# supranational/sppark

Hardware: AMD Instinct MI355X
Metric: MSM points/sec (BLS12-381 G1, 2^26 points) (higher is better)
Workload: dtype u32

## Files before the change

### sppark_amd/csrc/ec/xyzzx_dev.hpp

```cpp
#pragma once
#include "../ff/montx_dev.hpp"
#include "xyzz_dev.hpp"

namespace sppark_amd {

template<class FP> struct field_is_internal { static constexpr bool value = false; };
template<class P, int LB> struct field_is_internal<montx_dev<P, LB>> { static constexpr bool value = true; };
template<class FP> struct field_is_montx { static constexpr bool value = false; };
template<class P, int LB> struct field_is_montx<montx_dev<P, LB>> { static constexpr bool value = true; };

template<class P, int LB> struct affine_loader<montx_dev<P, LB>> {
    typedef montx_dev<P, LB> F;
    static constexpr unsigned RAW = 2 * F::NL * 4;
    static constexpr unsigned STRIDE = RAW <= 64 ? 64 : RAW <= 128 ? 128 : ((RAW + 15) / 16) * 16;
    template<bool FLAGGED>
    SPPARK_DEVFN static affine_dev<F> load(const unsigned char* base, size_t idx, unsigned)
    {
        const uint4* q = reinterpret_cast<const uint4*>(base + idx * (size_t)STRIDE);
        u32 w[(RAW + 15) / 16 * 4];
        #pragma unroll
        for (unsigned i = 0; i < (RAW + 15) / 16; i++) { uint4 v = q[i]; w[4*i] = v.x; w[4*i+1] = v.y; w[4*i+2] = v.z; w[4*i+3] = v.w; }
        affine_dev<F> a;
        a.X = F::from_wire(w); a.Y = F::from_wire(w + F::NL);
        a.inf = (a.X.l[F::NL - 1] >> 31) != 0;
        a.X.l[F::NL - 1] &= 0x7fffffffu;
        return a;
    }
    template<bool FLAGGED>
    SPPARK_DEVFN static void convert(unsigned char* dst, const unsigned char* src, size_t idx, unsigned stride)
    {
        typedef mont_dev<P> S;
        u32 wx[S::N], wy[S::N];
        bool inf;
        if (!FLAGGED && (S::N % 2) == 0 && (stride & 15) == 0 && ((size_t)src & 15) == 0) {
            const uint4* q = reinterpret_cast<const uint4*>(src + idx * (size_t)stride);
            u32 w[2 * S::N];
            #pragma unroll
            for (int i = 0; i < S::N / 2; i++) { uint4 v = q[i]; w[4*i] = v.x; w[4*i+1] = v.y; w[4*i+2] = v.z; w[4*i+3] = v.w; }
            u32 any = 0;
            #pragma unroll
            for (int i = 0; i < S::N; i++) { wx[i] = w[i]; wy[i] = w[S::N + i]; any |= w[i] | w[S::N + i]; }
            inf = any == 0;
        } else {
            affine_dev<S> p = affine_loader<S>::template load<FLAGGED>(src, idx, stride);
            p.X.to_wire(wx); p.Y.to_wire(wy);
            inf = p.inf;
        }
        F x = F::from_std(wx), y = F::from_std(wy);
        u32 w[STRIDE / 4] = {};
        x.to_wire(w); y.to_wire(w + F::NL);
        if (inf) w[F::NL - 1] |= 0x80000000u;
        uint4* q = reinterpret_cast<uint4*>(dst + idx * (size_t)STRIDE);
        #pragma unroll
        for (unsigned i = 0; i < STRIDE / 16; i++) q[i] = make_uint4(w[4*i], w[4*i+1], w[4*i+2], w[4*i+3]);
    }
};

template<class P, int LB> struct xyzz_dev<montx_dev<P, LB>> {
    typedef montx_dev<P, LB> F;
    F X, Y, ZZZ, ZZ;
    static constexpr bool TIGHT = F::TIGHT;
    static constexpr int BX = TIGHT ? 1 : 6;
    static constexpr int BX2 = TIGHT ? 1 : 4;
    SPPARK_DEVFN static F keep_x(const F& x3) { if constexpr (TIGHT) return x3.norm(); else return x3; }
    SPPARK_DEVFN static F minus_y(const F& y) { if constexpr (TIGHT) return F::template neg<4, 2>(y); else return F::template neg<6, 4>(y); }

    SPPARK_DEVFN bool is_inf() const { return ZZ.limbs_all_zero(); }
    SPPARK_DEVFN void set_inf() { X = F::zero(); Y = F::zero(); ZZZ = F::zero(); ZZ = F::zero(); }

    SPPARK_DEVFN void set(const affine_dev<F>& p, bool negate)
    {
        if (p.inf) { set_inf(); return; }
        X = p.X; Y = negate ? F::template neg<3>(p.Y) : p.Y;
        ZZZ = F::one(); ZZ = F::one();
    }

    SPPARK_DEVFN void madd(const affine_dev<F>& p, bool negate)
    {
        if (p.inf) return;
        if (is_inf()) { set(p, negate); return; }

        F U2, S2;
        F::template mul2<true, true>(U2, S2, p.X, ZZ, p.Y, ZZZ);
        if (negate) S2 = F::template neg<3>(S2);
        F Pd = F::template sub<11, BX>(U2, X).norm();
        F Rd;
        if constexpr (TIGHT) Rd = F::template sub<4, 2>(S2, Y).norm(); else Rd = F::template sub<6, 4>(S2, Y).norm();

        if (!Pd.template is_zero_mod<13>()) {
            F PP, RR, PPP, Q;
            F::sqr2(PP, RR, Pd, Rd);
            F::template mul2<true, false>(PPP, Q, Pd, PP, X, PP);
            F T   = PPP + Q + Q;
            F X3  = keep_x(F::template sub<8, 3>(RR, T));
            F D   = F::template sub<11, BX>(Q, X3);
            F nY  = minus_y(Y);
            Y   = F::mul_add(D, Rd, nY, PPP);
            F::template mul2<true, true>(ZZ, ZZZ, ZZ, PP, ZZZ, PPP);
            X = X3;
        } else if (Rd.template is_zero_mod<9>()) {
            F y2 = negate ? F::template neg<3>(p.Y).norm() : p.Y;
            dbl_affine(p.X, y2);
        } else {
            set_inf();
        }
    }

    SPPARK_DEVFN void add(const xyzz_dev& q)
    {
        if (q.is_inf()) return;
        if (is_inf()) { *this = q; return; }

        F U1 = X * q.ZZ;
        F S1 = Y * q.ZZZ;
        F U2 = q.X * ZZ;
        F S2 = q.Y * ZZZ;
        F Pd = F::template sub<3>(U2, U1).norm();
        F Rd = F::template sub<3>(S2, S1).norm();

        if (!Pd.template is_zero_mod<5>()) {
            F PP  = Pd.sqr();
            F PPP = Pd * PP;
            F Q   = U1 * PP;
            F T   = PPP + Q + Q;
            F X3  = keep_x(F::template sub<8, 3>(Rd.sqr(), T));
            F D   = F::template sub<11, BX>(Q, X3);
            Y   = F::mul_add(D, Rd, F::template neg<3>(S1), PPP);
            ZZ  = (ZZ * PP) * q.ZZ;
            ZZZ = (ZZZ * PPP) * q.ZZZ;
            X = X3;
        } else if (Rd.template is_zero_mod<5>()) {
            xyzz_dev t = *this;
            dbl_outlined(t);
            *this = t;
        } else {
            set_inf();
        }
    }

    SPPARK_DEVFN void add_pairs(const xyzz_dev& q)
    {
        if (q.is_inf()) return;
        if (is_inf()) { *this = q; return; }
        F U1, S1, U2, S2;
        F::mul2(U1, S1, X, q.ZZ, Y, q.ZZZ);
        F::mul2(U2, S2, q.X, ZZ, q.Y, ZZZ);
        F Pd = F::template sub<3>(U2, U1).norm();
        F Rd = F::template sub<3>(S2, S1).norm();
        if (!Pd.template is_zero_mod<5>()) {
            F PP, RR, PPP, Q, t0, t1;
            F::sqr2(PP, RR, Pd, Rd);
            F::template mul2<true, true>(PPP, Q, Pd, PP, U1, PP);
            F T   = PPP + Q + Q;
            F X3  = keep_x(F::template sub<8, 3>(RR, T));
            F D   = F::template sub<11, BX>(Q, X3);
            Y   = F::mul_add(D, Rd, F::template neg<3>(S1), PPP);
            F::template mul2<true, true>(t0, t1, ZZ, PP, ZZZ, PPP);
            F::template mul2<true, true>(ZZ, ZZZ, t0, q.ZZ, t1, q.ZZZ);
            X = X3;
        } else if (Rd.template is_zero_mod<5>()) {
            xyzz_dev t = *this;
            dbl_outlined(t);
            *this = t;
        } else {
            set_inf();
        }
    }
    SPPARK_DEVFN void dbl_pairs()
    {
        if (is_inf()) return;
        F Yn = Y.norm(), Xn = X.norm();
        F U = (Yn + Yn).norm();
        F V, M, W, S, M3s;
        F::sqr2(V, M, U, Xn);
        F::template mul2<true, true>(W, S, U, V, Xn, V);
        F M3 = (M + M + M).norm();
        M3s = M3.sqr();
        F X3 = keep_x(F::template sub<5, 2>(M3s, S + S));
        F D  = F::template sub<8, BX2>(S, X3);
        Y = F::mul_add(D, M3, F::template neg<3>(W), Yn);
        F::template mul2<true, true>(ZZ, ZZZ, ZZ, V, ZZZ, W);
        X = X3;
    }

#if defined(SPPARK_HOST_EMULATION)
    static void dbl_outlined(xyzz_dev& t) { t.dbl(); }
#else
    __device__ __noinline__ static void dbl_outlined(xyzz_dev& t) { t.dbl(); }
#endif

    SPPARK_DEVFN void dbl()
    {
        if (is_inf()) return;
        F Yn = Y.norm(), Xn = X.norm();
        F U = (Yn + Yn).norm();
        F V = U.sqr();
        F W = U * V;
        F S = Xn * V;
        F M = Xn.sqr();
        F M3 = (M + M + M).norm();
        F X3 = keep_x(F::template sub<5, 2>(M3.sqr(), S + S));
        F D  = F::template sub<8, BX2>(S, X3);
        Y = F::mul_add(D, M3, F::template neg<3>(W), Yn);
        ZZ = ZZ * V; ZZZ = ZZZ * W;
        X = X3;
    }

    typedef xyzz_mem<F::N> mem_t;

    SPPARK_DEVFN void store(mem_t* dst) const
    {
        constexpr int N = F::N;
        u32 s[4 * N];
        X.to_wire(s); Y.to_wire(s + N); ZZZ.to_wire(s + 2 * N); ZZ.to_wire(s + 3 * N);
        uint4* d = reinterpret_cast<uint4*>(dst);
        #pragma unroll
        for (int i = 0; i < N; i++) d[i] = make_uint4(s[4*i], s[4*i+1], s[4*i+2], s[4*i+3]);
    }
    SPPARK_DEVFN static xyzz_dev load(const mem_t* src)
    {
        constexpr int N = F::N;
        u32 d[4 * N];
        const uint4* q = reinterpret_cast<const uint4*>(src);
        #pragma unroll
        for (int i = 0; i < N; i++) { uint4 w = q[i]; d[4*i] = w.x; d[4*i+1] = w.y; d[4*i+2] = w.z; d[4*i+3] = w.w; }
        xyzz_dev r;
        r.X = F::from_wire(d); r.Y = F::from_wire(d + N); r.ZZZ = F::from_wire(d + 2 * N); r.ZZ = F::from_wire(d + 3 * N);
        return r;
    }

    SPPARK_DEVFN void store_std(xyzz_mem<P::N>* dst) const
    {
        constexpr int N = P::N;
        u32 s[4 * N];
        if (is_inf()) { for (int i = 0; i < 4 * N; i++) s[i] = 0; }
        else { X.to_std(s); Y.to_std(s + N); ZZZ.to_std(s + 2 * N); ZZ.to_std(s + 3 * N); }
        uint4* d = reinterpret_cast<uint4*>(dst);
        #pragma unroll
        for (int i = 0; i < N; i++) d[i] = make_uint4(s[4*i], s[4*i+1], s[4*i+2], s[4*i+3]);
    }

private:
    SPPARK_DEVFN void dbl_affine(const F& x, const F& y)
    {
        F U = (y + y).norm();
        F V = U.sqr();
        F W = U * V;
        F S = x * V;
        F M = x.sqr();
        F M3 = (M + M + M).norm();
        F X3 = keep_x(F::template sub<5, 2>(M3.sqr(), S + S));
        F D  = F::template sub<8, BX2>(S, X3);
        Y = F::mul_add(D, M3, F::template neg<3>(W), y);
        X = X3; ZZ = V; ZZZ = W;
    }
};

}
```

### sppark_amd/csrc/msm/msm_kernels.hpp

```cpp
#pragma once
#include "../ec/xyzz_dev.hpp"
#include "../ec/xyzzx_dev.hpp"

namespace sppark_amd {

static constexpr u32 KEY_NONE = 0xffffffffu;


__host__ __device__ inline unsigned window_len(unsigned w, unsigned nwins, unsigned nbits)
{   return nbits / nwins + (w < nbits % nwins ? 1u : 0u);   }

template<class LimbFn>
SPPARK_DEVFN void recode_digits(u32* digits, size_t n, size_t i, LimbFn limb, bool flip,
                                unsigned nwins, unsigned nbits, unsigned w_begin = 0, unsigned w_count = ~0u)
{
    u32 carry = 0;
    const unsigned w_end = w_count > nwins - w_begin ? nwins : w_begin + w_count;
    for (unsigned w = 0, bit = 0; w < w_end; w++) {
        const unsigned len = window_len(w, nwins, nbits);
        const u32 half = 1u << (len - 1), full = 1u << len, mask = full - 1;
        const unsigned li = bit >> 5, sh = bit & 31;
        bit += len;
        u64 two = limb(li) | ((u64)limb(li + 1) << 32);
        u32 d = ((u32)(two >> sh) & mask) + carry;
        bool minus = d > half;
        carry = minus;
        d = minus ? full - d : d;
        if (w >= w_begin) digits[(size_t)(w - w_begin) * n + i] = d ? (d | ((u32)(minus != flip) << 31)) : 0;
    }
}

template<class FR>
SPPARK_DEVFN FR load_scalar_abs(const u32* scalars, size_t i, int mont, bool& flip)
{
    constexpr int N = FR::N;
    FR s;
    const uint4* src = reinterpret_cast<const uint4*>(scalars + i * N);
    #pragma unroll
    for (int k = 0; k < N / 4; k++) {
        uint4 q = src[k];
        s.v[4*k] = q.x; s.v[4*k+1] = q.y; s.v[4*k+2] = q.z; s.v[4*k+3] = q.w;
    }
    if (mont) s = s.from();
    FR neg = FR::modulus_minus(s);
    u32 bw = 0;
    #pragma unroll
    for (int k = 0; k < N; k++) (void)__builtin_subc(neg.v[k], s.v[k], bw, &bw);
    flip = bw != 0;
    return FR::select(flip, neg, s);
}

template<class FR>
__global__ __launch_bounds__(256)
void k_breakdown(u32* __restrict__ digits, const u32* __restrict__ scalars,
                 unsigned n, unsigned nwins, unsigned nbits, int mont, unsigned w_begin, unsigned w_count)
{
    constexpr int N = FR::N;
    __shared__ u32 limbs[N + 2][256];
    const unsigned tid = threadIdx.x;
    for (unsigned i = blockIdx.x * 256 + tid; i < n; i += gridDim.x * 256) {
        bool flip;
        FR s = load_scalar_abs<FR>(scalars, i, mont, flip);
        #pragma unroll
        for (int k = 0; k < N; k++) limbs[k][tid] = s.v[k];
        limbs[N][tid] = 0; limbs[N + 1][tid] = 0;
        recode_digits(digits, n, i, [&](unsigned k) { return limbs[k][tid]; }, flip, nwins, nbits, w_begin, w_count);
    }
}

template<class FP, bool FLAGGED>
SPPARK_DEVFN void accumulate_chunk(xyzz_mem<FP::N>* buckets, u32* rec_key, xyzz_mem<FP::N>* rec_pt,
                                   const unsigned char* points, unsigned stride,
                                   const u32* sorted, const u32* off,
                                   unsigned n, unsigned NB, unsigned L, unsigned chunks_per_win,
                                   unsigned chunk, unsigned w_local, unsigned w_base = 0)
{
    if (chunk >= chunks_per_win) return;
    const unsigned w = w_base + w_local;
    const size_t rec0 = ((size_t)w * chunks_per_win + chunk) * 2;
    const u32* o = off + (size_t)w_local * (NB + 1);
    const unsigned total = o[NB];
    unsigned p = chunk * L;
    if (p >= total) { rec_key[rec0] = KEY_NONE; rec_key[rec0 + 1] = KEY_NONE; return; }
    const unsigned end = total < p + L ? total : p + L;

    unsigned lo = 0, hi = NB;
    while (hi - lo > 1) {
        unsigned mid = (lo + hi) >> 1;
        if (o[mid] <= p) lo = mid; else hi = mid;
    }
    unsigned b = lo, next = o[b + 1];

    const u32* src = sorted + (size_t)w_local * n;
    xyzz_dev<FP> acc;
    bool first_run = true;
    u32 slot0_key = KEY_NONE;

    u32 e = src[p];
    affine_dev<FP> pt = load_affine<FP, FLAGGED>(points, e & 0x7fffffffu, stride);
    acc.set(pt, e >> 31);
    constexpr bool PREFETCH = field_is_montx<FP>::value;
    u32 e_next = 0, e_next2 = 0;
    affine_dev<FP> pt_next = pt;
    if (PREFETCH && p + 1 < end) { e_next = src[p + 1]; pt_next = load_affine<FP, FLAGGED>(points, e_next & 0x7fffffffu, stride); }
    if (PREFETCH && p + 2 < end) e_next2 = src[p + 2];
    for (p++; p < end; p++) {
        if (PREFETCH) {
            e = e_next; pt = pt_next;
            if (p + 1 < end) { e_next = e_next2; pt_next = load_affine<FP, FLAGGED>(points, e_next & 0x7fffffffu, stride); }
            if (p + 2 < end) e_next2 = src[p + 2];
        } else {
            e = src[p];
            pt = load_affine<FP, FLAGGED>(points, e & 0x7fffffffu, stride);
        }
        if (p == next) {
            const u32 key = w * NB + b;
            if (first_run) { acc.store(&rec_pt[rec0]); slot0_key = key; first_run = false; }
            else           acc.store(&buckets[key]);
            do { b++; next = o[b + 1]; } while (p == next);
            acc.set(pt, e >> 31);
        } else {
            acc.madd(pt, e >> 31);
        }
    }
    const u32 key = w * NB + b;
    if (first_run) { acc.store(&rec_pt[rec0]); rec_key[rec0] = key; rec_key[rec0 + 1] = KEY_NONE; }
    else           { acc.store(&rec_pt[rec0 + 1]); rec_key[rec0] = slot0_key; rec_key[rec0 + 1] = key; }
}

#ifndef SPPARK_G2_TWO_WAVES_MAX_N
# define SPPARK_G2_TWO_WAVES_MAX_N 20
#endif
template<class FP, bool FLAGGED>
__global__ __launch_bounds__(256, (field_is_internal<FP>::value && FP::N <= 10) ? 3 : (field_is_internal<FP>::value && FP::N <= SPPARK_G2_TWO_WAVES_MAX_N) ? 2 : 1)
void k_accumulate(xyzz_mem<FP::N>* __restrict__ buckets,
                  u32* __restrict__ rec_key, xyzz_mem<FP::N>* __restrict__ rec_pt,
                  const unsigned char* __restrict__ points, unsigned stride,
                  const u32* __restrict__ sorted, const u32* __restrict__ off,
                  unsigned n, unsigned NB, unsigned L, unsigned chunks_per_win, unsigned w_base)
{
    accumulate_chunk<FP, FLAGGED>(buckets, rec_key, rec_pt, points, stride, sorted, off, n, NB, L,
                                  chunks_per_win, blockIdx.x * blockDim.x + threadIdx.x, blockIdx.y, w_base);
}

template<class FP, bool FLAGGED>
SPPARK_DEVFN void bitmap_accumulate_item(u32* rec_key, xyzz_mem<FP::N>* rec_pt,
                                         const unsigned char* points, unsigned stride, unsigned npoints,
                                         const u32* bitmap, const u32* refmap, unsigned span_words, size_t t)
{
    const size_t nwords = ((size_t)npoints + 31) / 32;
    const size_t w0 = t * span_words;
    if (w0 >= nwords) return;
    xyzz_dev<FP> acc; acc.set_inf();
    for (size_t w = w0; w < w0 + span_words && w < nwords; w++) {
        u32 bits = bitmap[w], refs = refmap ? refmap[w] : 0;
        bits ^= refs; refs &= bits;
        if (w == nwords - 1 && (npoints & 31)) bits &= (1u << (npoints & 31)) - 1;
        while (bits) {
            const unsigned k = __builtin_ctz(bits);
            bits &= bits - 1;
            affine_dev<FP> p = load_affine<FP, FLAGGED>(points, w * 32 + k, stride);
            acc.madd(p, (refs >> k) & 1);
        }
    }
    acc.store(&rec_pt[t]); rec_key[t] = 0;
}
template<class FP, bool FLAGGED>
__global__ __launch_bounds__(256)
void k_bitmap_accumulate(u32* __restrict__ rec_key, xyzz_mem<FP::N>* __restrict__ rec_pt,
                         const unsigned char* __restrict__ points, unsigned stride, unsigned npoints,
                         const u32* __restrict__ bitmap, const u32* __restrict__ refmap, unsigned span_words)
{
    bitmap_accumulate_item<FP, FLAGGED>(rec_key, rec_pt, points, stride, npoints, bitmap, refmap, span_words,
                                        (size_t)blockIdx.x * blockDim.x + threadIdx.x);
}

static constexpr unsigned JOIN_WALK = 8;
template<class FP> SPPARK_DEVFN void bucket_add(xyzz_dev<FP>& a, const xyzz_dev<FP>& b);
template<class FP> SPPARK_DEVFN void bucket_add_fast(xyzz_dev<FP>& a, const xyzz_dev<FP>& b);

template<class FP>
SPPARK_DEVFN void join_runs_item(xyzz_mem<FP::N>* buckets, u32* out_key, const u32* in_key,
                                 const xyzz_mem<FP::N>* in_pt, unsigned nrec, u32* any_long, size_t t)
{
    size_t job_h[2], job_e[2]; u32 job_k[2]; unsigned njobs = 0;
    for (unsigned s = 0; s < 2; s++) {
        if (t == 0 && s == 0) continue;
        const size_t q = 2 * t - 1 + s;
        if (q >= nrec) break;
        const u32 k = in_key[q];
        if (k == KEY_NONE) { out_key[q] = KEY_NONE; continue; }
        size_t h = q; bool is_long = false;
        for (size_t i = q, none = 0; i-- > 0;) {
            const u32 ki = in_key[i];
            if (ki == KEY_NONE) { if (++none == 2) break; continue; }
            none = 0;
            if (ki != k) break;
            h = i;
            if (q - h > JOIN_WALK) { is_long = true; break; }
        }
        size_t e = h;
        if (!is_long) {
            bool ended = false;
            size_t i = h + 1;
            for (unsigned none = 0; i < nrec && i <= h + JOIN_WALK; i++) {
                const u32 ki = in_key[i];
                if (ki == KEY_NONE) { if (++none == 2) { ended = true; break; } continue; }
                none = 0;
                if (ki != k) { ended = true; break; }
                e = i;
            }
            if (i >= nrec) ended = true;
            is_long = !ended;
        }
        if (is_long) { out_key[q] = k; *any_long = 1; continue; }
        out_key[q] = KEY_NONE;
        if (q == h) { job_h[njobs] = h; job_e[njobs] = e; job_k[njobs] = k; njobs++; }
    }
    for (unsigned j = 0; j < njobs; j++) {
        const size_t h = job_h[j], e = job_e[j]; const u32 k = job_k[j];
        xyzz_dev<FP> acc = xyzz_dev<FP>::load(&in_pt[h]);
        for (size_t i = h + 1; i <= e; i++)
            if (in_key[i] == k) bucket_add<FP>(acc, xyzz_dev<FP>::load(&in_pt[i]));
        acc.store(&buckets[k]);
    }
}

template<class FP>
SPPARK_DEVFN void reduce_runs_chunk(xyzz_mem<FP::N>* buckets, u32* out_key, xyzz_mem<FP::N>* out_pt,
                                    const u32* in_key, const xyzz_mem<FP::N>* in_pt,
                                    unsigned nrec, unsigned F, unsigned nthreads, int last, unsigned t)
{
    if (t >= nthreads) return;
    const unsigned lo = t * F, hi = nrec < lo + F ? nrec : lo + F;
    const size_t rec0 = (size_t)t * 2;

    xyzz_dev<FP> acc;
    u32 cur = KEY_NONE, slot0_key = KEY_NONE;
    bool first_run = true;

    for (unsigned r = lo; r < hi; r++) {
        const u32 k = in_key[r];
        if (k == KEY_NONE) continue;
        if (k == cur) {
            bucket_add_fast<FP>(acc, xyzz_dev<FP>::load(&in_pt[r]));
        } else {
            if (cur != KEY_NONE) {
                if (first_run && !last) { acc.store(&out_pt[rec0]); slot0_key = cur; }
                else                    acc.store(&buckets[cur]);
                first_run = false;
            }
            cur = k;
            acc = xyzz_dev<FP>::load(&in_pt[r]);
        }
    }
    if (last) {
        if (cur != KEY_NONE) acc.store(&buckets[cur]);
        return;
    }
    if (cur == KEY_NONE)      { out_key[rec0] = KEY_NONE; out_key[rec0 + 1] = KEY_NONE; }
    else if (first_run)       { acc.store(&out_pt[rec0]); out_key[rec0] = cur; out_key[rec0 + 1] = KEY_NONE; }
    else                      { acc.store(&out_pt[rec0 + 1]); out_key[rec0] = slot0_key; out_key[rec0 + 1] = cur; }
}

template<class FP>
__global__ __launch_bounds__(256)
void k_reduce_runs(xyzz_mem<FP::N>* __restrict__ buckets,
                   u32* __restrict__ out_key, xyzz_mem<FP::N>* __restrict__ out_pt,
                   const u32* __restrict__ in_key, const xyzz_mem<FP::N>* __restrict__ in_pt,
                   unsigned nrec, unsigned F, unsigned nthreads, int last, const u32* __restrict__ skip)
{
    if (skip != nullptr && *skip == 0) return;
    reduce_runs_chunk<FP>(buckets, out_key, out_pt, in_key, in_pt, nrec, F, nthreads, last,
                          blockIdx.x * blockDim.x + threadIdx.x);
}

static constexpr unsigned REDUCE_TAIL_NT = 256;
template<class FP>
__global__ __launch_bounds__(REDUCE_TAIL_NT)
void k_reduce_tail(xyzz_mem<FP::N>* __restrict__ buckets, u32* key0, xyzz_mem<FP::N>* pt0, u32* key1, xyzz_mem<FP::N>* pt1,
                   unsigned nrec, unsigned F, const u32* __restrict__ skip)
{
    if (skip != nullptr && *skip == 0) return;
    u32 *ik = key0, *ok = key1; xyzz_mem<FP::N> *ip = pt0, *op = pt1;
    for (;;) {
        const unsigned nthreads = (nrec + F - 1) / F;
        const int last = nthreads == 1;
        reduce_runs_chunk<FP>(buckets, ok, op, ik, ip, nrec, F, nthreads, last, threadIdx.x);
        if (last) break;
        __threadfence_block();
        __syncthreads();
        nrec = 2 * nthreads;
        u32* tk = ik; ik = ok; ok = tk;
        xyzz_mem<FP::N>* tp = ip; ip = op; op = tp;
    }
}

template<class FP>
__global__ __launch_bounds__(256, 2)
void k_join_runs(xyzz_mem<FP::N>* __restrict__ buckets, u32* __restrict__ out_key, const u32* __restrict__ in_key,
                 const xyzz_mem<FP::N>* __restrict__ in_pt, unsigned nrec, u32* __restrict__ any_long)
{
    join_runs_item<FP>(buckets, out_key, in_key, in_pt, nrec, any_long, (size_t)blockIdx.x * blockDim.x + threadIdx.x);
}

#if defined(SPPARK_HOST_EMULATION)
# define SPPARK_OUTLINED inline
#else
# define SPPARK_OUTLINED __device__ __noinline__
#endif
template<class FP> SPPARK_OUTLINED void xyzz_add_outlined(xyzz_dev<FP>& a, const xyzz_dev<FP>& b) { a.add(b); }
template<class FP> SPPARK_OUTLINED void xyzz_dbl_outlined(xyzz_dev<FP>& a) { a.dbl(); }
template<class FP> SPPARK_DEVFN void bucket_add(xyzz_dev<FP>& a, const xyzz_dev<FP>& b)
{   if constexpr (FP::N > 16) xyzz_add_outlined<FP>(a, b); else a.add(b);   }
template<class FP> SPPARK_DEVFN void bucket_dbl(xyzz_dev<FP>& a)
{   if constexpr (FP::N > 16) xyzz_dbl_outlined<FP>(a); else a.dbl();   }
template<class FP> SPPARK_DEVFN void bucket_add_fast(xyzz_dev<FP>& a, const xyzz_dev<FP>& b)
{   if constexpr (field_is_montx<FP>::value) a.add_pairs(b); else bucket_add<FP>(a, b);   }
template<class FP> SPPARK_DEVFN void bucket_dbl_fast(xyzz_dev<FP>& a)
{   if constexpr (field_is_montx<FP>::value) a.dbl_pairs(); else bucket_dbl<FP>(a);   }

template<class FP>
SPPARK_DEVFN xyzz_dev<FP> bucket_load(const xyzz_mem<FP::N>* row, const u32* o, unsigned b)
{
    if (o != nullptr && o[b + 1] == o[b]) { xyzz_dev<FP> z; z.set_inf(); return z; }
    return xyzz_dev<FP>::load(&row[b]);
}
template<class FP, bool LAT = false>
SPPARK_DEVFN void bucket_level1_item(xyzz_mem<FP::N>* A, xyzz_mem<FP::N>* Wt, const xyzz_mem<FP::N>* buckets,
                                     unsigned NB, unsigned K, unsigned nwins, size_t id, const u32* off = nullptr)
{
    const unsigned nchunks = NB / K;
    if (id >= (size_t)nwins * nchunks) return;
    const unsigned w = id / nchunks, u = id % nchunks;
    const xyzz_mem<FP::N>* row = buckets + (size_t)w * NB + (size_t)u * K;
    const u32* o = off ? off + (size_t)w * (NB + 1) + (size_t)u * K : nullptr;
    xyzz_dev<FP> acc = bucket_load<FP>(row, o, K - 1), ret = acc;
    for (unsigned j = K - 1; j--;) {
        if (LAT) { bucket_add_fast<FP>(acc, bucket_load<FP>(row, o, j)); bucket_add_fast<FP>(ret, acc); }
        else     { bucket_add<FP>(acc, bucket_load<FP>(row, o, j)); bucket_add<FP>(ret, acc); }
    }
    acc.store(&A[id]); ret.store(&Wt[id]);
}

template<class FP>
__global__ __launch_bounds__(256, 2)
void k_bucket_level1(xyzz_mem<FP::N>* __restrict__ A, xyzz_mem<FP::N>* __restrict__ Wt,
                     const xyzz_mem<FP::N>* __restrict__ buckets, unsigned NB, unsigned K, unsigned nwins,
                     const u32* __restrict__ off)
{   bucket_level1_item<FP>(A, Wt, buckets, NB, K, nwins, (size_t)blockIdx.x * blockDim.x + threadIdx.x, off);   }
template<class FP>
__global__ __launch_bounds__(256)
void k_bucket_level1_lat(xyzz_mem<FP::N>* __restrict__ A, xyzz_mem<FP::N>* __restrict__ Wt,
                         const xyzz_mem<FP::N>* __restrict__ buckets, unsigned NB, unsigned K, unsigned nwins,
                         const u32* __restrict__ off)
{   bucket_level1_item<FP, true>(A, Wt, buckets, NB, K, nwins, (size_t)blockIdx.x * blockDim.x + threadIdx.x, off);   }

template<class FP, bool LAT = false>
SPPARK_DEVFN void bucket_levelN_item(xyzz_mem<FP::N>* A2, xyzz_mem<FP::N>* Wt2,
                                     const xyzz_mem<FP::N>* A1, const xyzz_mem<FP::N>* Wt1,
                                     unsigned nitems, unsigned K, unsigned lgG, unsigned nwins, size_t id)
{
    const unsigned nchunks = nitems / K;
    if (id >= (size_t)nwins * nchunks) return;
    const unsigned w = id / nchunks, u = id % nchunks;
    const size_t base = (size_t)w * nitems + (size_t)u * K;
    xyzz_dev<FP> acc, r, sw;
    acc.set_inf(); r.set_inf();
    sw = xyzz_dev<FP>::load(&Wt1[base]);
    auto add = [](xyzz_dev<FP>& a, const xyzz_dev<FP>& b) { if (LAT) bucket_add_fast<FP>(a, b); else bucket_add<FP>(a, b); };
    for (unsigned j = K - 1; j >= 1; j--) {
        add(acc, xyzz_dev<FP>::load(&A1[base + j]));
        add(r, acc);
        add(sw, xyzz_dev<FP>::load(&Wt1[base + j]));
    }
    add(acc, xyzz_dev<FP>::load(&A1[base]));
    for (unsigned k = 0; k < lgG; k++) { if (LAT) bucket_dbl_fast<FP>(r); else bucket_dbl<FP>(r); }
    add(sw, r);
    acc.store(&A2[id]); sw.store(&Wt2[id]);
}

template<class FP>
__global__ __launch_bounds__(256, 2)
void k_bucket_levelN(xyzz_mem<FP::N>* __restrict__ A2, xyzz_mem<FP::N>* __restrict__ Wt2,
                     const xyzz_mem<FP::N>* __restrict__ A1, const xyzz_mem<FP::N>* __restrict__ Wt1,
                     unsigned nitems, unsigned K, unsigned lgG, unsigned nwins)
{   bucket_levelN_item<FP>(A2, Wt2, A1, Wt1, nitems, K, lgG, nwins, (size_t)blockIdx.x * blockDim.x + threadIdx.x);   }
template<class FP>
__global__ __launch_bounds__(256)
void k_bucket_levelN_lat(xyzz_mem<FP::N>* __restrict__ A2, xyzz_mem<FP::N>* __restrict__ Wt2,
                         const xyzz_mem<FP::N>* __restrict__ A1, const xyzz_mem<FP::N>* __restrict__ Wt1,
                         unsigned nitems, unsigned K, unsigned lgG, unsigned nwins)
{   bucket_levelN_item<FP, true>(A2, Wt2, A1, Wt1, nitems, K, lgG, nwins, (size_t)blockIdx.x * blockDim.x + threadIdx.x);   }

static constexpr unsigned BUCKET_TOP_MAX = 4096, BUCKET_TOP_NT = 256;

template<class FP>
SPPARK_DEVFN void lds_tree_sum(xyzz_dev<FP>& acc, xyzz_mem<FP::N>* img, unsigned tid, unsigned nt)
{
    for (unsigned s = nt >> 1; s >= 1; s >>= 1) {
        if (tid >= s && tid < 2 * s) acc.store(&img[tid]);
        __syncthreads();
        if (tid < s) bucket_add_fast<FP>(acc, xyzz_dev<FP>::load(&img[tid + s]));
        __syncthreads();
    }
}

template<class FP>
SPPARK_DEVFN xyzz_dev<FP> bucket_top_gather(const xyzz_mem<FP::N>* A, const xyzz_mem<FP::N>* Wt,
                                            unsigned nitems, unsigned m, unsigned b, unsigned w, unsigned tid, unsigned nt)
{
    const xyzz_mem<FP::N>* src = (b == m ? Wt : A) + (size_t)w * nitems;
    unsigned lgI = 0;
    while ((nt << lgI) < nitems) lgI++;
    const unsigned p = b >= m ? 0 : (b < m - lgI ? b : m - lgI);
    const unsigned lo = tid & ((1u << p) - 1), hi = tid >> p;
    xyzz_dev<FP> acc; acc.set_inf();
    #pragma unroll 1
    for (unsigned i = 0; i < (1u << lgI); i++) {
        const unsigned j = lo | (i << p) | (hi << (p + lgI));
        if (j < nitems && (b == m || ((j >> b) & 1))) bucket_add_fast<FP>(acc, xyzz_dev<FP>::load(&src[j]));
    }
    return acc;
}
template<class FP>
SPPARK_DEVFN void bucket_top_finish(xyzz_dev<FP>& acc, xyzz_mem<FP::N>* parts, unsigned m, unsigned lgG, unsigned b, unsigned w)
{
    if (b < m) {
        #pragma unroll 1
        for (unsigned k = 0; k < b + lgG; k++) bucket_dbl_fast<FP>(acc);
    }
    acc.store(&parts[(size_t)w * (m + 1) + b]);
}
struct top_piece { unsigned b, sub, nsub; };
SPPARK_DEVFN top_piece bucket_top_piece(unsigned q, unsigned m, unsigned sb, unsigned sp)
{
    top_piece t;
    if (q < m * sb) { t.b = q / sb; t.sub = q % sb; t.nsub = sb; }
    else            { t.b = m; t.sub = q - m * sb; t.nsub = sp; }
    return t;
}
static inline void bucket_top_cut(unsigned nitems, unsigned nt, unsigned& sb, unsigned& sp)
{
    sb = 1;
    sp = nitems >= 16 * nt ? 2 : 1;
}

template<class FP>
SPPARK_DEVFN xyzz_dev<FP> bucket_top_sum_gather(const xyzz_mem<FP::N>* parts, unsigned m, unsigned w, unsigned tid)
{
    xyzz_dev<FP> acc; acc.set_inf();
    if (tid <= m) acc = xyzz_dev<FP>::load(&parts[(size_t)w * (m + 1) + tid]);
    return acc;
}

static constexpr unsigned SMALL_SUMS_MAX_NB = 256;
SPPARK_DEVFN unsigned small_sums_member(unsigned b, unsigned m, unsigned t)
{   return b >= m ? (1u << m) : ((((t >> b) << 1) | 1u) << b) | (t & ((1u << b) - 1u));   }

template<class FP>
SPPARK_DEVFN xyzz_dev<FP> small_sums_gather(const xyzz_mem<FP::N>* buckets, const u32* off, unsigned NB, unsigned m,
                                            unsigned b, unsigned w, unsigned t)
{
    xyzz_dev<FP> r; r.set_inf();
    if (t >= (b >= m ? 1u : NB / 2)) return r;
    const unsigned j = small_sums_member(b, m, t) - 1;
    return bucket_load<FP>(buckets + (size_t)w * NB, off + (size_t)w * (NB + 1), j);
}

template<class FP>
__global__ __launch_bounds__(BUCKET_TOP_NT, 2)
void k_bucket_top_bits(xyzz_mem<FP::N>* __restrict__ parts, const xyzz_mem<FP::N>* __restrict__ A,
                       const xyzz_mem<FP::N>* __restrict__ Wt, unsigned nitems, unsigned m, unsigned lgG)
{
    extern __shared__ unsigned char top_lds[];
    xyzz_mem<FP::N>* img = reinterpret_cast<xyzz_mem<FP::N>*>(top_lds);
    const unsigned b = blockIdx.x, w = blockIdx.y, tid = threadIdx.x;
    xyzz_dev<FP> acc = bucket_top_gather<FP>(A, Wt, nitems, m, b, w, tid, BUCKET_TOP_NT);
    lds_tree_sum<FP>(acc, img, tid, BUCKET_TOP_NT);
    if (tid == 0) bucket_top_finish<FP>(acc, parts, m, lgG, b, w);
}

template<class FP>
__global__ __launch_bounds__(32)
void k_bucket_top_sum(xyzz_mem<FP::N>* __restrict__ out, const xyzz_mem<FP::N>* __restrict__ parts, unsigned m)
{
    extern __shared__ unsigned char top_lds[];
    xyzz_mem<FP::N>* img = reinterpret_cast<xyzz_mem<FP::N>*>(top_lds);
    const unsigned w = blockIdx.x, tid = threadIdx.x;
    xyzz_dev<FP> acc = bucket_top_sum_gather<FP>(parts, m, w, tid);
    lds_tree_sum<FP>(acc, img, tid, 32);
    if (tid == 0) acc.store(&out[w]);
}

template<class FP>
SPPARK_DEVFN constexpr unsigned convert_lds_stride(unsigned raw) { return (raw / 4) % 8 == 0 ? raw + 16 : raw; }
template<class FP, bool FLAGGED>
__global__ __launch_bounds__(256)
void k_convert_points_staged(unsigned char* __restrict__ dst, const unsigned char* __restrict__ src, unsigned n)
{
    typedef affine_loader<FP> AL;
    constexpr unsigned IN = 2 * FP::NW * 4 + (FLAGGED ? 8 : 0), OUT = AL::STRIDE;
    constexpr unsigned IN_L = FLAGGED ? IN : convert_lds_stride<FP>(IN), OUT_L = convert_lds_stride<FP>(OUT);
    static_assert(IN % 8 == 0 && (256 * IN) % 16 == 0 && OUT % 16 == 0, "8 / 16-byte pieces");
    constexpr unsigned LDS_BYTES = 256 * (IN_L > OUT_L ? IN_L : OUT_L) + 16;
    __shared__ uint4 img[LDS_BYTES / 16];
    unsigned char* lds = reinterpret_cast<unsigned char*>(img);
    const unsigned tid = threadIdx.x;
    const size_t p0 = (size_t)blockIdx.x * 256;
    const unsigned cnt = n - p0 < 256 ? (unsigned)(n - p0) : 256u;
    const unsigned char* gin = src + p0 * IN;
    const unsigned bytes = cnt * IN;
    #pragma unroll
    for (unsigned it = 0; it < (256 * IN / 16 + 255) / 256; it++) {
        const unsigned g = it * 256 + tid, at = g * 16;
        if (at + 16 <= bytes) {
            const uint4 v = *reinterpret_cast<const uint4*>(gin + at);
            if (FLAGGED) *reinterpret_cast<uint4*>(lds + at) = v;
            else         *reinterpret_cast<uint4*>(lds + (g / (IN / 16)) * IN_L + (g % (IN / 16)) * 16) = v;
        } else if (FLAGGED && at + 8 <= bytes) {
            *reinterpret_cast<uint2*>(lds + at) = *reinterpret_cast<const uint2*>(gin + at);
        }
    }
    __syncthreads();
    u32 w[OUT / 4] = {};
    if (tid < cnt) {
        u32 in[IN / 4];
        if (FLAGGED) {
            #pragma unroll
            for (unsigned j = 0; j < IN / 8; j++) {
                const uint2 v = *reinterpret_cast<const uint2*>(lds + tid * IN_L + j * 8);
                in[2*j] = v.x; in[2*j+1] = v.y;
            }
        } else {
            #pragma unroll
            for (unsigned j = 0; j < IN / 16; j++) {
                const uint4 v = *reinterpret_cast<const uint4*>(lds + tid * IN_L + j * 16);
                in[4*j] = v.x; in[4*j+1] = v.y; in[4*j+2] = v.z; in[4*j+3] = v.w;
            }
        }
        bool inf;
        if (FLAGGED) inf = (in[2 * FP::NW] & 1u) != 0;
        else {
            u32 any = 0;
            #pragma unroll
            for (unsigned i = 0; i < 2 * FP::NW; i++) any |= in[i];
            inf = any == 0;
        }
        const FP x = FP::from_std(in), y = FP::from_std(in + FP::NW);
        x.to_wire(w); y.to_wire(w + FP::NL);
        if (inf) w[FP::NL - 1] |= 0x80000000u;
    }
    __syncthreads();
    if (tid < cnt) {
        #pragma unroll
        for (unsigned j = 0; j < OUT / 16; j++)
            *reinterpret_cast<uint4*>(lds + tid * OUT_L + j * 16) = make_uint4(w[4*j], w[4*j+1], w[4*j+2], w[4*j+3]);
    }
    __syncthreads();
    uint4* gout = reinterpret_cast<uint4*>(dst + p0 * OUT);
    #pragma unroll
    for (unsigned it = 0; it < OUT / 16; it++) {
        const unsigned g = it * 256 + tid;
        if (g < cnt * (OUT / 16)) gout[g] = *reinterpret_cast<const uint4*>(lds + (g / (OUT / 16)) * OUT_L + (g % (OUT / 16)) * 16);
    }
}


template<class FP, bool FLAGGED>
__global__ __launch_bounds__(256)
void k_convert_points(unsigned char* __restrict__ dst, const unsigned char* __restrict__ src, unsigned n, unsigned stride)
{
    size_t i = (size_t)blockIdx.x * blockDim.x + threadIdx.x;
    if (i < n) affine_loader<FP>::template convert<FLAGGED>(dst, src, i, stride);
}

template<class FP>
SPPARK_DEVFN void fixed_base_table_item(unsigned char* table, unsigned n, unsigned nwins, unsigned nbits, size_t i)
{
    typedef affine_loader<FP> AL;
    constexpr unsigned GROUP = 8;
    if (i >= n) return;
    affine_dev<FP> p = load_affine<FP, false>(table, i, 0);
    xyzz_dev<FP> acc; acc.set(p, false);
    #pragma unroll 1
    for (unsigned j0 = 1; j0 < nwins; j0 += GROUP) {
        const unsigned cnt = nwins - j0 < GROUP ? nwins - j0 : GROUP;
        xyzz_dev<FP> sv[GROUP]; FP pre[GROUP]; bool inf[GROUP];
        FP run = FP::one();
        #pragma unroll 1
        for (unsigned g = 0; g < cnt; g++) {
            #pragma unroll 1
            for (unsigned k = 0; k < window_len(j0 + g - 1, nwins, nbits); k++) acc.dbl();
            const FP zz = acc.ZZ * acc.ZZZ;
            inf[g] = acc.is_inf() || zz.template is_zero_mod<2>();
            if (inf[g]) acc.set_inf();
            sv[g] = acc; pre[g] = run;
            if (!inf[g]) run = run * zz;
        }
        FP inv = run.inverse();
        #pragma unroll 1
        for (unsigned g = cnt; g--;) {
            u32 w[AL::STRIDE / 4] = {};
            if (inf[g]) {
                w[FP::NL - 1] = 0x80000000u;
            } else {
                const FP zz = sv[g].ZZ * sv[g].ZZZ;
                const FP iz = inv * pre[g];
                inv = inv * zz;
                const FP x = sv[g].X * (iz * sv[g].ZZZ), y = sv[g].Y * (iz * sv[g].ZZ);
                x.to_wire(w); y.to_wire(w + FP::NL);
            }
            uint4* q = reinterpret_cast<uint4*>(table + ((size_t)(j0 + g) * n + i) * (size_t)AL::STRIDE);
            #pragma unroll
            for (unsigned k = 0; k < AL::STRIDE / 16; k++) q[k] = make_uint4(w[4*k], w[4*k+1], w[4*k+2], w[4*k+3]);
        }
    }
}
template<class FP>
__global__ __launch_bounds__(256)
void k_fixed_base_table(unsigned char* __restrict__ table, unsigned n, unsigned nwins, unsigned nbits)
{   fixed_base_table_item<FP>(table, n, nwins, nbits, (size_t)blockIdx.x * blockDim.x + threadIdx.x);   }

template<class FP, int STD_WORDS>
__global__ __launch_bounds__(64)
void k_finalize(xyzz_mem<STD_WORDS>* __restrict__ out, const xyzz_mem<FP::N>* __restrict__ in, unsigned count)
{
    unsigned i = blockIdx.x * blockDim.x + threadIdx.x;
    if (i < count) xyzz_dev<FP>::load(&in[i]).store_std(&out[i]);
}

}
```

Measured before the change: 522.5 million.

## Prefetch raw point words and bucket offsets in accumulate, bitmask empty buckets

Splits the montx affine load into a raw-word gather and a separate decode. The accumulate loop now prefetches only raw words one point ahead, with a volatile asm pin so the loads are issued early, and it clamps indices so the loop body has no branches. Bucket boundary offsets are also prefetched one bucket ahead, and a bucket change becomes set_inf followed by a uniform madd instead of a separate set path. Level-1 bucket reduction precomputes an empty-bucket bitmask from the offsets instead of reading two offsets per bucket load. The added madd from infinity and the extra clamped loads are extra work, and keeping the raw words live raises register pressure.

```diff
diff --git a/sppark_amd/csrc/ec/xyzzx_dev.hpp b/sppark_amd/csrc/ec/xyzzx_dev.hpp
--- a/sppark_amd/csrc/ec/xyzzx_dev.hpp
+++ b/sppark_amd/csrc/ec/xyzzx_dev.hpp
@@ -13,19 +13,35 @@
     typedef montx_dev<P, LB> F;
     static constexpr unsigned RAW = 2 * F::NL * 4;
     static constexpr unsigned STRIDE = RAW <= 64 ? 64 : RAW <= 128 ? 128 : ((RAW + 15) / 16) * 16;
-    template<bool FLAGGED>
-    SPPARK_DEVFN static affine_dev<F> load(const unsigned char* base, size_t idx, unsigned)
+    struct raw_t {
+        u32 w[(RAW + 15) / 16 * 4];
+        SPPARK_DEVFN void landed() const
+        {
+#if defined(__HIP_DEVICE_COMPILE__)
+            #pragma unroll
+            for (unsigned i = 0; i < (RAW + 15) / 16 * 4; i++) asm volatile("" :: "v"(w[i]));
+#endif
+        }
+    };
+    SPPARK_DEVFN static raw_t load_raw(const unsigned char* base, size_t idx)
     {
         const uint4* q = reinterpret_cast<const uint4*>(base + idx * (size_t)STRIDE);
-        u32 w[(RAW + 15) / 16 * 4];
-        #pragma unroll
-        for (unsigned i = 0; i < (RAW + 15) / 16; i++) { uint4 v = q[i]; w[4*i] = v.x; w[4*i+1] = v.y; w[4*i+2] = v.z; w[4*i+3] = v.w; }
+        raw_t r;
+        #pragma unroll
+        for (unsigned i = 0; i < (RAW + 15) / 16; i++) { uint4 v = q[i]; r.w[4*i] = v.x; r.w[4*i+1] = v.y; r.w[4*i+2] = v.z; r.w[4*i+3] = v.w; }
+        return r;
+    }
+    SPPARK_DEVFN static affine_dev<F> decode(const raw_t& r)
+    {
         affine_dev<F> a;
-        a.X = F::from_wire(w); a.Y = F::from_wire(w + F::NL);
+        a.X = F::from_wire(r.w); a.Y = F::from_wire(r.w + F::NL);
         a.inf = (a.X.l[F::NL - 1] >> 31) != 0;
         a.X.l[F::NL - 1] &= 0x7fffffffu;
         return a;
     }
+    template<bool FLAGGED>
+    SPPARK_DEVFN static affine_dev<F> load(const unsigned char* base, size_t idx, unsigned)
+    {   return decode(load_raw(base, idx));   }
     template<bool FLAGGED>
     SPPARK_DEVFN static void convert(unsigned char* dst, const unsigned char* src, size_t idx, unsigned stride)
     {
diff --git a/sppark_amd/csrc/msm/msm_kernels.hpp b/sppark_amd/csrc/msm/msm_kernels.hpp
--- a/sppark_amd/csrc/msm/msm_kernels.hpp
+++ b/sppark_amd/csrc/msm/msm_kernels.hpp
@@ -68,6 +68,9 @@
     }
 }
 
+template<class FP, bool ON> struct gather_raw { struct type {}; };
+template<class FP> struct gather_raw<FP, true> { typedef typename affine_loader<FP>::raw_t type; };
+
 template<class FP, bool FLAGGED>
 SPPARK_DEVFN void accumulate_chunk(xyzz_mem<FP::N>* buckets, u32* rec_key, xyzz_mem<FP::N>* rec_pt,
                                    const unsigned char* points, unsigned stride,
@@ -89,7 +92,7 @@
         unsigned mid = (lo + hi) >> 1;
         if (o[mid] <= p) lo = mid; else hi = mid;
     }
-    unsigned b = lo, next = o[b + 1];
+    unsigned b = lo, next = o[b + 1], next2 = o[b + 2 < NB ? b + 2 : NB];
 
     const u32* src = sorted + (size_t)w_local * n;
     xyzz_dev<FP> acc;
@@ -101,14 +104,17 @@
     acc.set(pt, e >> 31);
     constexpr bool PREFETCH = field_is_montx<FP>::value;
     u32 e_next = 0, e_next2 = 0;
-    affine_dev<FP> pt_next = pt;
-    if (PREFETCH && p + 1 < end) { e_next = src[p + 1]; pt_next = load_affine<FP, FLAGGED>(points, e_next & 0x7fffffffu, stride); }
-    if (PREFETCH && p + 2 < end) e_next2 = src[p + 2];
+    typename gather_raw<FP, PREFETCH>::type raw_next = {};
+    const unsigned last = end - 1;
+    if constexpr (PREFETCH) {
+        e_next = src[p + 1 < last ? p + 1 : last];
+        raw_next = affine_loader<FP>::load_raw(points, e_next & 0x7fffffffu);
+        e_next2 = src[p + 2 < last ? p + 2 : last];
+    }
+    if constexpr (PREFETCH) raw_next.landed();
     for (p++; p < end; p++) {
-        if (PREFETCH) {
-            e = e_next; pt = pt_next;
-            if (p + 1 < end) { e_next = e_next2; pt_next = load_affine<FP, FLAGGED>(points, e_next & 0x7fffffffu, stride); }
-            if (p + 2 < end) e_next2 = src[p + 2];
+        if constexpr (PREFETCH) {
+            e = e_next; pt = affine_loader<FP>::decode(raw_next);
         } else {
             e = src[p];
             pt = load_affine<FP, FLAGGED>(points, e & 0x7fffffffu, stride);
@@ -117,11 +123,17 @@
             const u32 key = w * NB + b;
             if (first_run) { acc.store(&rec_pt[rec0]); slot0_key = key; first_run = false; }
             else           acc.store(&buckets[key]);
-            do { b++; next = o[b + 1]; } while (p == next);
-            acc.set(pt, e >> 31);
-        } else {
-            acc.madd(pt, e >> 31);
-        }
+            b++; next = next2;
+            if (p == next) do { b++; next = o[b + 1]; } while (p == next);
+            next2 = o[b + 2 < NB ? b + 2 : NB];
+            acc.set_inf();
+        }
+        if constexpr (PREFETCH) {
+            e_next = e_next2;
+            raw_next = affine_loader<FP>::load_raw(points, e_next & 0x7fffffffu);
+            e_next2 = src[p + 2 < last ? p + 2 : last];
+        }
+        acc.madd(pt, e >> 31);
     }
     const u32 key = w * NB + b;
     if (first_run) { acc.store(&rec_pt[rec0]); rec_key[rec0] = key; rec_key[rec0 + 1] = KEY_NONE; }
@@ -335,10 +347,25 @@
     const unsigned w = id / nchunks, u = id % nchunks;
     const xyzz_mem<FP::N>* row = buckets + (size_t)w * NB + (size_t)u * K;
     const u32* o = off ? off + (size_t)w * (NB + 1) + (size_t)u * K : nullptr;
-    xyzz_dev<FP> acc = bucket_load<FP>(row, o, K - 1), ret = acc;
+    constexpr unsigned LEVEL1_BITS = 16;
+    const bool bits = o != nullptr && K <= LEVEL1_BITS;
+    u32 empty = 0;
+    if (bits) {
+        u32 ov[LEVEL1_BITS + 1];
+        #pragma unroll
+        for (unsigned j = 0; j <= LEVEL1_BITS; j++) ov[j] = o[j < K ? j : K];
+        #pragma unroll
+        for (unsigned j = 0; j < LEVEL1_BITS; j++) empty |= (u32)(ov[j + 1] == ov[j]) << j;
+    }
+    auto load = [&](unsigned j) {
+        if (!bits) return bucket_load<FP>(row, o, j);
+        if ((empty >> j) & 1) { xyzz_dev<FP> z; z.set_inf(); return z; }
+        return xyzz_dev<FP>::load(&row[j]);
+    };
+    xyzz_dev<FP> acc = load(K - 1), ret = acc;
     for (unsigned j = K - 1; j--;) {
-        if (LAT) { bucket_add_fast<FP>(acc, bucket_load<FP>(row, o, j)); bucket_add_fast<FP>(ret, acc); }
-        else     { bucket_add<FP>(acc, bucket_load<FP>(row, o, j)); bucket_add<FP>(ret, acc); }
+        if (LAT) { bucket_add_fast<FP>(acc, load(j)); bucket_add_fast<FP>(ret, acc); }
+        else     { bucket_add<FP>(acc, load(j)); bucket_add<FP>(ret, acc); }
     }
     acc.store(&A[id]); ret.store(&Wt[id]);
 }
```

Result: faster. 531.2 million (median of 6 runs) (+1.7%).
